# uc-vision/splat-trainer

Hardware: AMD Instinct MI355X
Metric: fwd+bwd Gaussians/s (higher is better)
Workload: dtype f32

## Files before the change

### splat-trainer_amd/csrc/ssim.hip

```cpp
#include "gsr_device.h"
#include "gsr_host.h"

namespace {

constexpr int TS = 32;
constexpr int HALO = 5;
constexpr int IN = TS + 2 * HALO;

struct Gauss11 {
  float w[11];
};

struct Strides {
  int64_t sB, sC, sH, sW;
};

__device__ __forceinline__ float clamp_keep_nan(float v, float lo, float hi) {
  return v < lo ? lo : (v > hi ? hi : v);
}

__device__ __forceinline__ float block_sum_256(float v, float* s_red) {
  v = gsr_wave_sum(v);
  const int wave = threadIdx.x >> 6;
  if ((threadIdx.x & 63) == 0) s_red[wave] = v;
  __syncthreads();
  return s_red[0] + s_red[1] + s_red[2] + s_red[3];
}

template <bool TRAIN>
__global__ __launch_bounds__(256) void ssim_fwd_kernel(const float* __restrict__ img1, const float* __restrict__ img2,
                                                       Strides st1, Strides st2, int C, int H, int W, int crop,
                                                       float C1, float C2, float inv_count, Gauss11 g,
                                                       float* __restrict__ block_sums, float* __restrict__ dm_dmu1,
                                                       float* __restrict__ dm_dm11, float* __restrict__ dm_dm12,
                                                       float lo = -INFINITY, float hi = INFINITY) {
  __shared__ float s_x[IN][IN + 1], s_y[IN][IN + 1];
  __shared__ float s_h[5][IN][TS + 1];
  __shared__ float s_red[4];
  const int plane = blockIdx.z, b = plane / C, c = plane % C;
  const int x0 = blockIdx.x * TS, y0 = blockIdx.y * TS;
  const float* p1 = img1 + b * st1.sB + c * st1.sC;
  const float* p2 = img2 + b * st2.sB + c * st2.sC;
  const int cy = min(y0 + TS / 2, H - 1), cx = min(x0 + TS / 2, W - 1);
  float c1 = clamp_keep_nan(p1[cy * st1.sH + cx * st1.sW], lo, hi), c2 = p2[cy * st2.sH + cx * st2.sW];
  c1 = fabsf(c1) <= 3.0e38f ? c1 : 0.f;
  c2 = fabsf(c2) <= 3.0e38f ? c2 : 0.f;
  for (int i = threadIdx.x; i < IN * IN; i += 256) {
    const int ly = i / IN, lx = i % IN;
    const int gy = y0 + ly - HALO, gx = x0 + lx - HALO;
    const bool in = gy >= 0 && gy < H && gx >= 0 && gx < W;
    s_x[ly][lx] = in ? clamp_keep_nan(p1[gy * st1.sH + gx * st1.sW], lo, hi) - c1 : 0.f;
    s_y[ly][lx] = in ? p2[gy * st2.sH + gx * st2.sW] - c2 : 0.f;
  }
  __syncthreads();
  for (int i = threadIdx.x; i < IN * (TS / 4); i += 256) {
    const int ly = i / (TS / 4), lx = (i % (TS / 4)) * 4;
    float x[14], y[14], xx[14], yy[14], xy[14];
#pragma unroll
    for (int k = 0; k < 14; ++k) {
      x[k] = s_x[ly][lx + k]; y[k] = s_y[ly][lx + k];
      xx[k] = x[k] * x[k]; yy[k] = y[k] * y[k]; xy[k] = x[k] * y[k];
    }
#pragma unroll
    for (int o = 0; o < 4; ++o) {
      float a = 0.f, bb = 0.f, aa = 0.f, bb2 = 0.f, ab = 0.f;
#pragma unroll
      for (int k = 0; k < 11; ++k) {
        const float w = g.w[k];
        a += w * x[o + k]; bb += w * y[o + k]; aa += w * xx[o + k]; bb2 += w * yy[o + k]; ab += w * xy[o + k];
      }
      s_h[0][ly][lx + o] = a; s_h[1][ly][lx + o] = bb; s_h[2][ly][lx + o] = aa; s_h[3][ly][lx + o] = bb2;
      s_h[4][ly][lx + o] = ab;
    }
  }
  __syncthreads();
  const int tx = threadIdx.x & 31, tg = threadIdx.x >> 5;
  const int gx = x0 + tx;
  float acc[4][5];
#pragma unroll
  for (int o = 0; o < 4; ++o)
#pragma unroll
    for (int q = 0; q < 5; ++q) acc[o][q] = 0.f;
#pragma unroll
  for (int q = 0; q < 5; ++q) {
    float col[14];
#pragma unroll
    for (int k = 0; k < 14; ++k) col[k] = s_h[q][tg * 4 + k][tx];
#pragma unroll
    for (int o = 0; o < 4; ++o)
#pragma unroll
      for (int k = 0; k < 11; ++k) acc[o][q] += g.w[k] * col[o + k];
  }
  float local = 0.f;
  float out_x = 0.f;
#pragma unroll
  for (int k = 0; k < 11; ++k) out_x += (gx + k - HALO < 0 || gx + k - HALO >= W) ? g.w[k] : 0.f;
#pragma unroll
  for (int o = 0; o < 4; ++o) {
    const int gy = y0 + tg * 4 + o;
    float out_y = 0.f;
#pragma unroll
    for (int k = 0; k < 11; ++k) out_y += (gy + k - HALO < 0 || gy + k - HALO >= H) ? g.w[k] : 0.f;
    const float mass = (1.f - out_x) * (1.f - out_y), rest = out_x + (1.f - out_x) * out_y;
    const float n1 = acc[o][0], n2 = acc[o][1];
    const float mu1 = n1 + c1 * mass, mu2 = n2 + c2 * mass;
    const float s1 = (acc[o][2] - n1 * n1) + c1 * rest * (2.f * n1 + c1 * mass);
    const float s2 = (acc[o][3] - n2 * n2) + c2 * rest * (2.f * n2 + c2 * mass);
    const float s12 = (acc[o][4] - n1 * n2) + rest * (c2 * n1 + c1 * n2 + c1 * c2 * mass);
    const bool inside = gx < W && gy < H;
    const bool counted = inside && gx >= crop && gx < W - crop && gy >= crop && gy < H - crop;
    const float A1 = 2.f * mu1 * mu2 + C1, A2 = 2.f * s12 + C2;
    const float B1 = mu1 * mu1 + mu2 * mu2 + C1, B2 = s1 + s2 + C2;
    const float iB = 1.f / (B1 * B2);
    if (counted) local += A1 * A2 * iB;
    if (TRAIN && inside) {
      const float sc = counted ? inv_count : 0.f;
      const float d_mu1 = 2.f * mu2 * (A2 - A1) * iB - 2.f * mu1 * A1 * A2 * (B2 - B1) * iB * iB;
      const float d_m11 = -A1 * A2 * iB / B2;
      const float d_m12 = 2.f * A1 * iB;
      const int64_t oidx = ((int64_t)plane * H + gy) * W + gx;
      dm_dmu1[oidx] = sc * d_mu1; dm_dm11[oidx] = sc * d_m11; dm_dm12[oidx] = sc * d_m12;
    }
  }
  const float total = block_sum_256(local, s_red);
  if (threadIdx.x == 0)
    block_sums[(blockIdx.z * gridDim.y + blockIdx.y) * gridDim.x + blockIdx.x] = total;
}

__global__ __launch_bounds__(256) void ssim_finish_kernel(const float* __restrict__ block_sums, int n, float inv_count,
                                                          float* __restrict__ out) {
  __shared__ float s_red[4];
  float acc = 0.f;
  for (int i = threadIdx.x; i < n; i += 256) acc += block_sums[i];
  const float total = block_sum_256(acc, s_red);
  if (threadIdx.x == 0) out[0] = total * inv_count;
}

__global__ __launch_bounds__(256) void ssim_bwd_kernel(const float* __restrict__ img1, const float* __restrict__ img2,
                                                       Strides st1, Strides st2, Strides sto, int C, int H, int W,
                                                       Gauss11 g, const float* __restrict__ dm_dmu1,
                                                       const float* __restrict__ dm_dm11,
                                                       const float* __restrict__ dm_dm12,
                                                       const float* __restrict__ gscale_dev, float* __restrict__ dimg1,
                                                       float lo = -INFINITY, float hi = INFINITY) {
  __shared__ float s_in[3][IN][IN + 1];
  __shared__ float s_h[3][IN][TS + 1];
  const int plane = blockIdx.z, b = plane / C, c = plane % C;
  const int x0 = blockIdx.x * TS, y0 = blockIdx.y * TS;
  const int64_t pbase = (int64_t)plane * H * W;
  for (int i = threadIdx.x; i < IN * IN; i += 256) {
    const int ly = i / IN, lx = i % IN;
    const int gy = y0 + ly - HALO, gx = x0 + lx - HALO;
    const bool in = gy >= 0 && gy < H && gx >= 0 && gx < W;
    const int64_t o = pbase + (int64_t)gy * W + gx;
    s_in[0][ly][lx] = in ? dm_dmu1[o] : 0.f;
    s_in[1][ly][lx] = in ? dm_dm11[o] : 0.f;
    s_in[2][ly][lx] = in ? dm_dm12[o] : 0.f;
  }
  __syncthreads();
  for (int i = threadIdx.x; i < IN * (TS / 4); i += 256) {
    const int ly = i / (TS / 4), lx = (i % (TS / 4)) * 4;
#pragma unroll
    for (int q = 0; q < 3; ++q) {
      float v[14];
#pragma unroll
      for (int k = 0; k < 14; ++k) v[k] = s_in[q][ly][lx + k];
#pragma unroll
      for (int o = 0; o < 4; ++o) {
        float a = 0.f;
#pragma unroll
        for (int k = 0; k < 11; ++k) a += g.w[k] * v[o + k];
        s_h[q][ly][lx + o] = a;
      }
    }
  }
  __syncthreads();
  const int tx = threadIdx.x & 31, tg = threadIdx.x >> 5;
  const int gx = x0 + tx;
  float acc[4][3];
#pragma unroll
  for (int q = 0; q < 3; ++q) {
    float col[14];
#pragma unroll
    for (int k = 0; k < 14; ++k) col[k] = s_h[q][tg * 4 + k][tx];
#pragma unroll
    for (int o = 0; o < 4; ++o) {
      float a = 0.f;
#pragma unroll
      for (int k = 0; k < 11; ++k) a += g.w[k] * col[o + k];
      acc[o][q] = a;
    }
  }
  if (gx >= W) return;
  const float gs = gscale_dev ? gscale_dev[0] : 1.f;
#pragma unroll
  for (int o = 0; o < 4; ++o) {
    const int gy = y0 + tg * 4 + o;
    if (gy >= H) continue;
    const float x = clamp_keep_nan(img1[b * st1.sB + c * st1.sC + gy * st1.sH + gx * st1.sW], lo, hi);
    const float y = img2[b * st2.sB + c * st2.sC + gy * st2.sH + gx * st2.sW];
    dimg1[b * sto.sB + c * sto.sC + gy * sto.sH + gx * sto.sW] = gs * (acc[o][0] + 2.f * x * acc[o][1] + y * acc[o][2]);
  }
}

Gauss11 make_gauss() {
  Gauss11 g;
  double sum = 0.0, w[11];
  for (int i = 0; i < 11; ++i) { const double d = i - 5; w[i] = exp(-(d * d) / (2.0 * 1.5 * 1.5)); sum += w[i]; }
  for (int i = 0; i < 11; ++i) g.w[i] = (float)(w[i] / sum);
  return g;
}

constexpr int PL_THREADS = 256;
constexpr int PL_ITEMS = 8;

template <int KIND>
__global__ __launch_bounds__(PL_THREADS) void pixel_loss_fwd_kernel(const float* __restrict__ x,
                                                                    const float* __restrict__ t, int64_t n, float lo,
                                                                    float hi, float* __restrict__ block_sums) {
  __shared__ float s_w[PL_THREADS / 64];
  float acc = 0.f;
  for (int64_t i = ((int64_t)blockIdx.x * PL_THREADS + threadIdx.x) * 4; i < n; i += (int64_t)gridDim.x * PL_THREADS * 4) {
    float xv[4], tv[4];
    if (i + 3 < n) {
      const float4 a = *reinterpret_cast<const float4*>(x + i), b = *reinterpret_cast<const float4*>(t + i);
      xv[0] = a.x; xv[1] = a.y; xv[2] = a.z; xv[3] = a.w; tv[0] = b.x; tv[1] = b.y; tv[2] = b.z; tv[3] = b.w;
    } else {
#pragma unroll
      for (int k = 0; k < 4; ++k) { xv[k] = i + k < n ? x[i + k] : 0.f; tv[k] = i + k < n ? t[i + k] : clamp_keep_nan(0.f, lo, hi); }
    }
#pragma unroll
    for (int k = 0; k < 4; ++k) {
      const float d = clamp_keep_nan(xv[k], lo, hi) - tv[k];
      acc += KIND == 0 ? d * d : fabsf(d);
    }
  }
  acc = gsr_wave_sum(acc);
  if (gsr_lane() == 0) s_w[threadIdx.x >> 6] = acc;
  __syncthreads();
  if (threadIdx.x == 0) block_sums[blockIdx.x] = (s_w[0] + s_w[1]) + (s_w[2] + s_w[3]);
}

__global__ __launch_bounds__(256) void pixel_loss_finish_kernel(const float* __restrict__ block_sums, int blocks,
                                                                float inv_n, float* __restrict__ out) {
  __shared__ float s_w[4];
  float acc = 0.f;
  for (int b = threadIdx.x; b < blocks; b += 256) acc += block_sums[b];
  acc = gsr_wave_sum(acc);
  if (gsr_lane() == 0) s_w[threadIdx.x >> 6] = acc;
  __syncthreads();
  if (threadIdx.x == 0) out[0] = ((s_w[0] + s_w[1]) + (s_w[2] + s_w[3])) * inv_n;
}

template <int KIND>
__global__ __launch_bounds__(PL_THREADS) void pixel_loss_bwd_kernel(const float* __restrict__ x,
                                                                    const float* __restrict__ t, int64_t n, float lo,
                                                                    float hi, float inv_n,
                                                                    const float* __restrict__ grad_scale,
                                                                    float* __restrict__ dx) {
  const float gs = grad_scale[0] * inv_n;
  for (int64_t i = (int64_t)blockIdx.x * PL_THREADS + threadIdx.x; i < n; i += (int64_t)gridDim.x * PL_THREADS) {
    const float xv = x[i];
    const float d = clamp_keep_nan(xv, lo, hi) - t[i];
    const bool pass = xv >= lo && xv <= hi;
    const float g = KIND == 0 ? 2.f * d : (d > 0.f ? 1.f : (d < 0.f ? -1.f : 0.f));
    dx[i] = pass ? gs * g : 0.f;
  }
}

constexpr int ML_MAX_LEVELS = 4;

struct MsLevels {
  int n;
  int H[ML_MAX_LEVELS], W[ML_MAX_LEVELS];
  float* pred[ML_MAX_LEVELS];
  float* targ[ML_MAX_LEVELS];
  float* dlev[ML_MAX_LEVELS];
};

__global__ __launch_bounds__(256) void msloss_pyramid_kernel(const float* __restrict__ image,
                                                             const float* __restrict__ target, int C, MsLevels lv,
                                                             float lo, float hi, float* __restrict__ block_l1,
                                                             float* __restrict__ block_mse) {
  __shared__ float s_a[4], s_b[4];
  const int H = lv.H[0], W = lv.W[0];
  const int bw = (W + 7) / 8, bh = (H + 7) / 8;
  const int64_t id = (int64_t)blockIdx.x * 256 + threadIdx.x;
  float l1 = 0.f, mse = 0.f;
  if (id < (int64_t)bw * bh * C) {
    const int c = (int)(id % C);
    const int bx = (int)((id / C) % bw), by = (int)(id / ((int64_t)C * bw));
    float x1[4][4], t1[4][4];
#pragma unroll
    for (int j = 0; j < 4; ++j)
#pragma unroll
      for (int i = 0; i < 4; ++i) {
        float sx = 0.f, st = 0.f;
#pragma unroll
        for (int dy = 0; dy < 2; ++dy)
#pragma unroll
          for (int dx = 0; dx < 2; ++dx) {
            const int y = by * 8 + 2 * j + dy, x = bx * 8 + 2 * i + dx;
            if (y < H && x < W) {
              const int64_t o = ((int64_t)y * W + x) * C + c;
              const float xv = clamp_keep_nan(image[o], lo, hi), tv = target[o];
              const float d = xv - tv;
              l1 += fabsf(d);
              mse += d * d;
              sx += xv; st += tv;
            }
          }
        x1[j][i] = 0.25f * sx; t1[j][i] = 0.25f * st;
        const int y1 = by * 4 + j, xq = bx * 4 + i;
        if (lv.n > 1 && y1 < lv.H[1] && xq < lv.W[1]) {
          const int64_t o = ((int64_t)y1 * lv.W[1] + xq) * C + c;
          lv.pred[1][o] = x1[j][i]; lv.targ[1][o] = t1[j][i];
        }
      }
    if (lv.n > 2) {
      float x2[2][2], t2[2][2];
#pragma unroll
      for (int j = 0; j < 2; ++j)
#pragma unroll
        for (int i = 0; i < 2; ++i) {
          x2[j][i] = 0.25f * ((x1[2 * j][2 * i] + x1[2 * j][2 * i + 1]) + (x1[2 * j + 1][2 * i] + x1[2 * j + 1][2 * i + 1]));
          t2[j][i] = 0.25f * ((t1[2 * j][2 * i] + t1[2 * j][2 * i + 1]) + (t1[2 * j + 1][2 * i] + t1[2 * j + 1][2 * i + 1]));
          const int y2 = by * 2 + j, xq = bx * 2 + i;
          if (y2 < lv.H[2] && xq < lv.W[2]) {
            const int64_t o = ((int64_t)y2 * lv.W[2] + xq) * C + c;
            lv.pred[2][o] = x2[j][i]; lv.targ[2][o] = t2[j][i];
          }
        }
      if (lv.n > 3 && by < lv.H[3] && bx < lv.W[3]) {
        const int64_t o = ((int64_t)by * lv.W[3] + bx) * C + c;
        lv.pred[3][o] = 0.25f * ((x2[0][0] + x2[0][1]) + (x2[1][0] + x2[1][1]));
        lv.targ[3][o] = 0.25f * ((t2[0][0] + t2[0][1]) + (t2[1][0] + t2[1][1]));
      }
    }
  }
  l1 = gsr_wave_sum(l1);
  mse = gsr_wave_sum(mse);
  if (gsr_lane() == 0) { s_a[threadIdx.x >> 6] = l1; s_b[threadIdx.x >> 6] = mse; }
  __syncthreads();
  if (threadIdx.x == 0) {
    block_l1[blockIdx.x] = (s_a[0] + s_a[1]) + (s_a[2] + s_a[3]);
    block_mse[blockIdx.x] = (s_b[0] + s_b[1]) + (s_b[2] + s_b[3]);
  }
}

struct MsSums {
  const float* ssim[ML_MAX_LEVELS];
  int ssim_n[ML_MAX_LEVELS];
  float ssim_inv[ML_MAX_LEVELS];
  const float* l1;
  const float* mse;
  int pix_n;
  float pix_inv;
};

__global__ __launch_bounds__(256) void msloss_finish_kernel(MsSums sm, int levels, float w_l1, float w_mse, float w_ssim,
                                                            float* __restrict__ metrics_out) {
  __shared__ float s_red[4];
  float vals[2 + ML_MAX_LEVELS];
  float a = 0.f;
  for (int i = threadIdx.x; i < sm.pix_n; i += 256) a += sm.l1[i];
  vals[0] = block_sum_256(a, s_red) * sm.pix_inv;
  __syncthreads();
  a = 0.f;
  for (int i = threadIdx.x; i < sm.pix_n; i += 256) a += sm.mse[i];
  vals[1] = block_sum_256(a, s_red) * sm.pix_inv;
  __syncthreads();
  float ssim_loss = 0.f;
  for (int l = 0; l < levels; ++l) {
    a = 0.f;
    for (int i = threadIdx.x; i < sm.ssim_n[l]; i += 256) a += sm.ssim[l][i];
    vals[2 + l] = block_sum_256(a, s_red) * sm.ssim_inv[l];
    __syncthreads();
    ssim_loss += 1.f - vals[2 + l];
  }
  if (threadIdx.x == 0) {
    metrics_out[0] = vals[0] * w_l1 + vals[1] * w_mse + (ssim_loss / (float)levels) * w_ssim;
    for (int k = 0; k < 2 + levels; ++k) metrics_out[1 + k] = vals[k];
  }
}

__global__ __launch_bounds__(256) void msloss_combine_kernel(const float* __restrict__ image,
                                                             const float* __restrict__ target, int C, MsLevels lv,
                                                             float lo, float hi, float w_l1, float w_mse, float w_ssim,
                                                             const float* __restrict__ up, float* __restrict__ d_image) {
  const int H = lv.H[0], W = lv.W[0];
  const int64_t n = (int64_t)H * W * C;
  const float inv_n = 1.f / (float)n, gs = up[0], cs = -w_ssim / (float)lv.n;
  for (int64_t i = (int64_t)blockIdx.x * 256 + threadIdx.x; i < n; i += (int64_t)gridDim.x * 256) {
    const float xv = image[i];
    if (!(xv >= lo && xv <= hi)) { d_image[i] = 0.f; continue; }
    const int c = (int)(i % C);
    const int64_t p = i / C;
    const int x = (int)(p % W), y = (int)(p / W);
    const float d = xv - target[i];
    float g = w_l1 * inv_n * (d > 0.f ? 1.f : (d < 0.f ? -1.f : 0.f)) + w_mse * inv_n * 2.f * d;
    float s = d_image[i], sc = 0.25f;
#pragma unroll
    for (int l = 1; l < ML_MAX_LEVELS; ++l) {
      if (l < lv.n) {
        const int yl = y >> l, xl = x >> l;
        if (yl < lv.H[l] && xl < lv.W[l]) s += sc * lv.dlev[l][((int64_t)yl * lv.W[l] + xl) * C + c];
        sc *= 0.25f;
      }
    }
    d_image[i] = gs * (g + cs * s);
  }
}

struct MsPlan {
  MsLevels lv;
  size_t maps[ML_MAX_LEVELS];
  size_t sums[ML_MAX_LEVELS];
  int sums_n[ML_MAX_LEVELS];
  size_t pix_l1, pix_mse;
  int pix_blocks;
  size_t total;
};

MsPlan ms_plan(int H, int W, int C, int levels, uint8_t* base) {
  MsPlan p;
  size_t at = 0;
  auto take = [&](size_t bytes) { const size_t o = at; at = (at + bytes + 255) / 256 * 256; return o; };
  p.lv.n = levels;
  int h = H, w = W;
  for (int l = 0; l < ML_MAX_LEVELS; ++l) {
    p.lv.H[l] = p.lv.W[l] = 0;
    p.lv.pred[l] = p.lv.targ[l] = p.lv.dlev[l] = nullptr;
    p.maps[l] = p.sums[l] = 0; p.sums_n[l] = 0;
    if (l >= levels) continue;
    if (l > 0) { h /= 2; w /= 2; }
    p.lv.H[l] = h; p.lv.W[l] = w;
    const size_t plane = (size_t)h * w * C * sizeof(float);
    if (l > 0) {
      p.lv.pred[l] = reinterpret_cast<float*>(base + take(plane));
      p.lv.targ[l] = reinterpret_cast<float*>(base + take(plane));
      p.lv.dlev[l] = reinterpret_cast<float*>(base + take(plane));
    }
    p.maps[l] = take(3 * plane);
    p.sums_n[l] = ((w + TS - 1) / TS) * ((h + TS - 1) / TS) * C;
    p.sums[l] = take((size_t)p.sums_n[l] * sizeof(float));
  }
  const int64_t work = (int64_t)((W + 7) / 8) * ((H + 7) / 8) * C;
  p.pix_blocks = (int)((work + 255) / 256);
  p.pix_l1 = take((size_t)p.pix_blocks * sizeof(float));
  p.pix_mse = take((size_t)p.pix_blocks * sizeof(float));
  p.total = at;
  return p;
}

inline bool ms_args_ok(int H, int W, int C, int levels) {
  if (H <= 0 || W <= 0 || C < 1 || C > 4 || levels < 1 || levels > ML_MAX_LEVELS) return false;
  return (H >> (levels - 1)) > 10 && (W >> (levels - 1)) > 10;
}

}

extern "C" {

size_t gsr_ssim_workspace_bytes(int32_t B, int32_t C, int32_t H, int32_t W) {
  if (B <= 0 || C <= 0 || H <= 0 || W <= 0) return 256;
  const size_t blocks = (size_t)((W + TS - 1) / TS) * ((H + TS - 1) / TS) * B * C;
  return blocks * sizeof(float) + 256;
}

int gsr_ssim_forward(const float* img1, const float* img2, const int64_t* strides1_host, const int64_t* strides2_host,
                     int32_t B, int32_t C, int32_t H, int32_t W, int32_t crop, float* mean_out, float* dm_dmu1,
                     float* dm_dm11, float* dm_dm12, void* workspace, size_t workspace_bytes, void* stream_) {
  hipStream_t stream = gsr_stream(stream_);
  if (B <= 0 || C <= 0 || H <= 0 || W <= 0 || crop < 0 || !img1 || !img2 || !mean_out || !strides1_host || !strides2_host)
    return GSR_ERR_INVALID_ARGUMENT;
  if (W - 2 * crop <= 0 || H - 2 * crop <= 0) return GSR_ERR_INVALID_ARGUMENT;
  if (!workspace || workspace_bytes < gsr_ssim_workspace_bytes(B, C, H, W)) return GSR_ERR_WORKSPACE_TOO_SMALL;
  const bool train = dm_dmu1 && dm_dm11 && dm_dm12;
  const Strides s1 = {strides1_host[0], strides1_host[1], strides1_host[2], strides1_host[3]};
  const Strides s2 = {strides2_host[0], strides2_host[1], strides2_host[2], strides2_host[3]};
  const dim3 grid((W + TS - 1) / TS, (H + TS - 1) / TS, B * C);
  const int nblocks = grid.x * grid.y * grid.z;
  const float inv_count = 1.f / ((float)B * C * (H - 2 * crop) * (float)(W - 2 * crop));
  float* block_sums = reinterpret_cast<float*>(workspace);
  const Gauss11 g = make_gauss();
  gsr_pick_bool(train, [&](auto tr) {
    ssim_fwd_kernel<decltype(tr)::value><<<grid, 256, 0, stream>>>(
        img1, img2, s1, s2, C, H, W, crop, 0.01f * 0.01f, 0.03f * 0.03f, inv_count, g, block_sums,
        train ? dm_dmu1 : nullptr, train ? dm_dm11 : nullptr, train ? dm_dm12 : nullptr);
  });
  GSR_CHECK_LAUNCH();
  ssim_finish_kernel<<<1, 256, 0, stream>>>(block_sums, nblocks, inv_count, mean_out);
  GSR_CHECK_LAUNCH();
  return GSR_OK;
}

int gsr_ssim_backward(const float* img1, const float* img2, const int64_t* strides1_host, const int64_t* strides2_host,
                      const int64_t* strides_out_host, int32_t B, int32_t C, int32_t H, int32_t W, const float* dm_dmu1,
                      const float* dm_dm11, const float* dm_dm12, const float* grad_scale_dev, float* d_img1,
                      void* stream_) {
  hipStream_t stream = gsr_stream(stream_);
  if (B <= 0 || C <= 0 || H <= 0 || W <= 0 || !img1 || !img2 || !dm_dmu1 || !dm_dm11 || !dm_dm12 || !grad_scale_dev ||
      !d_img1 || !strides1_host || !strides2_host || !strides_out_host)
    return GSR_ERR_INVALID_ARGUMENT;
  const Strides s1 = {strides1_host[0], strides1_host[1], strides1_host[2], strides1_host[3]};
  const Strides s2 = {strides2_host[0], strides2_host[1], strides2_host[2], strides2_host[3]};
  const Strides so = {strides_out_host[0], strides_out_host[1], strides_out_host[2], strides_out_host[3]};
  const dim3 grid((W + TS - 1) / TS, (H + TS - 1) / TS, B * C);
  ssim_bwd_kernel<<<grid, 256, 0, stream>>>(img1, img2, s1, s2, so, C, H, W, make_gauss(), dm_dmu1, dm_dm11, dm_dm12,
                                           grad_scale_dev, d_img1);
  GSR_CHECK_LAUNCH();
  return GSR_OK;
}

size_t gsr_msloss_workspace_bytes(int32_t H, int32_t W, int32_t C, int32_t levels) {
  if (!ms_args_ok(H, W, C, levels)) return 256;
  return ms_plan(H, W, C, levels, nullptr).total + 256;
}

int gsr_msloss_forward(const float* image, const float* target, int32_t H, int32_t W, int32_t C, int32_t levels,
                       float w_l1, float w_mse, float w_ssim, float lo, float hi, float* metrics_out, void* workspace,
                       size_t workspace_bytes, void* stream_) {
  hipStream_t stream = gsr_stream(stream_);
  if (!ms_args_ok(H, W, C, levels) || !image || !target || !metrics_out || !(lo <= hi)) return GSR_ERR_INVALID_ARGUMENT;
  if (!workspace || workspace_bytes < gsr_msloss_workspace_bytes(H, W, C, levels)) return GSR_ERR_WORKSPACE_TOO_SMALL;
  uint8_t* base = reinterpret_cast<uint8_t*>(workspace);
  const MsPlan p = ms_plan(H, W, C, levels, base);
  msloss_pyramid_kernel<<<p.pix_blocks, 256, 0, stream>>>(image, target, C, p.lv, lo, hi,
                                                         reinterpret_cast<float*>(base + p.pix_l1),
                                                         reinterpret_cast<float*>(base + p.pix_mse));
  GSR_CHECK_LAUNCH();
  const Gauss11 g = make_gauss();
  MsSums sm;
  for (int l = 0; l < ML_MAX_LEVELS; ++l) { sm.ssim[l] = nullptr; sm.ssim_n[l] = 0; sm.ssim_inv[l] = 0.f; }
  for (int l = 0; l < levels; ++l) {
    const int h = p.lv.H[l], w = p.lv.W[l];
    const Strides st = {0, 1, (int64_t)w * C, C};
    const float* x = l ? p.lv.pred[l] : image;
    const float* t = l ? p.lv.targ[l] : target;
    const dim3 grid((w + TS - 1) / TS, (h + TS - 1) / TS, C);
    const float inv_count = 1.f / ((float)C * (h - 10) * (float)(w - 10));
    float* maps = reinterpret_cast<float*>(base + p.maps[l]);
    const size_t plane = (size_t)h * w * C;
    ssim_fwd_kernel<true><<<grid, 256, 0, stream>>>(x, t, st, st, C, h, w, 5, 0.01f * 0.01f, 0.03f * 0.03f, inv_count, g,
                                                   reinterpret_cast<float*>(base + p.sums[l]), maps, maps + plane,
                                                   maps + 2 * plane, l ? -INFINITY : lo, l ? INFINITY : hi);
    GSR_CHECK_LAUNCH();
    sm.ssim[l] = reinterpret_cast<const float*>(base + p.sums[l]);
    sm.ssim_n[l] = p.sums_n[l];
    sm.ssim_inv[l] = inv_count;
  }
  sm.l1 = reinterpret_cast<const float*>(base + p.pix_l1);
  sm.mse = reinterpret_cast<const float*>(base + p.pix_mse);
  sm.pix_n = p.pix_blocks;
  sm.pix_inv = 1.f / ((float)H * (float)W * (float)C);
  msloss_finish_kernel<<<1, 256, 0, stream>>>(sm, levels, w_l1, w_mse, w_ssim, metrics_out);
  GSR_CHECK_LAUNCH();
  return GSR_OK;
}

int gsr_msloss_backward(const float* image, const float* target, int32_t H, int32_t W, int32_t C, int32_t levels,
                        float w_l1, float w_mse, float w_ssim, float lo, float hi, const float* grad_scale_dev,
                        void* workspace, size_t workspace_bytes, float* d_image, void* stream_) {
  hipStream_t stream = gsr_stream(stream_);
  if (!ms_args_ok(H, W, C, levels) || !image || !target || !grad_scale_dev || !d_image) return GSR_ERR_INVALID_ARGUMENT;
  if (!workspace || workspace_bytes < gsr_msloss_workspace_bytes(H, W, C, levels)) return GSR_ERR_WORKSPACE_TOO_SMALL;
  uint8_t* base = reinterpret_cast<uint8_t*>(workspace);
  const MsPlan p = ms_plan(H, W, C, levels, base);
  const Gauss11 g = make_gauss();
  for (int l = 0; l < levels; ++l) {
    const int h = p.lv.H[l], w = p.lv.W[l];
    const Strides st = {0, 1, (int64_t)w * C, C};
    const float* x = l ? p.lv.pred[l] : image;
    const float* t = l ? p.lv.targ[l] : target;
    const float* maps = reinterpret_cast<const float*>(base + p.maps[l]);
    const size_t plane = (size_t)h * w * C;
    const dim3 grid((w + TS - 1) / TS, (h + TS - 1) / TS, C);
    ssim_bwd_kernel<<<grid, 256, 0, stream>>>(x, t, st, st, st, C, h, w, g, maps, maps + plane, maps + 2 * plane, nullptr,
                                             l ? p.lv.dlev[l] : d_image, l ? -INFINITY : lo, l ? INFINITY : hi);
    GSR_CHECK_LAUNCH();
  }
  const int64_t n = (int64_t)H * W * C;
  const int64_t want = (n + 255) / 256;
  msloss_combine_kernel<<<(int)(want < 16384 ? want : 16384), 256, 0, stream>>>(image, target, C, p.lv, lo, hi, w_l1, w_mse,
                                                                              w_ssim, grad_scale_dev, d_image);
  GSR_CHECK_LAUNCH();
  return GSR_OK;
}

size_t gsr_pixel_loss_workspace_bytes(int64_t n) {
  const int64_t blocks = (n + (int64_t)PL_THREADS * 4 - 1) / ((int64_t)PL_THREADS * 4);
  return (size_t)(blocks < 1024 ? (blocks < 1 ? 1 : blocks) : 1024) * sizeof(float) + 256;
}

int gsr_pixel_loss_forward(const float* image, const float* target, int64_t n, int32_t kind, float lo, float hi,
                           float* loss_out, void* workspace, size_t workspace_bytes, void* stream_) {
  hipStream_t stream = gsr_stream(stream_);
  if (n <= 0 || !image || !target || !loss_out || (kind != 0 && kind != 1) || !(lo <= hi)) return GSR_ERR_INVALID_ARGUMENT;
  if (!workspace || workspace_bytes < gsr_pixel_loss_workspace_bytes(n)) return GSR_ERR_WORKSPACE_TOO_SMALL;
  if ((reinterpret_cast<uintptr_t>(image) | reinterpret_cast<uintptr_t>(target)) & 15) return GSR_ERR_INVALID_ARGUMENT;
  const int64_t want = (n + (int64_t)PL_THREADS * 4 - 1) / ((int64_t)PL_THREADS * 4);
  const int blocks = (int)(want < 1024 ? want : 1024);
  float* sums = reinterpret_cast<float*>(workspace);
  gsr_pick<0, 1>(kind, [&](auto k) {
    pixel_loss_fwd_kernel<decltype(k)::value><<<blocks, PL_THREADS, 0, stream>>>(image, target, n, lo, hi, sums);
  });
  pixel_loss_finish_kernel<<<1, 256, 0, stream>>>(sums, blocks, 1.f / (float)n, loss_out);
  GSR_CHECK_LAUNCH();
  return GSR_OK;
}

int gsr_pixel_loss_backward(const float* image, const float* target, int64_t n, int32_t kind, float lo, float hi,
                            const float* grad_scale_dev, float* d_image, void* stream_) {
  hipStream_t stream = gsr_stream(stream_);
  if (n <= 0 || !image || !target || !grad_scale_dev || !d_image || (kind != 0 && kind != 1)) return GSR_ERR_INVALID_ARGUMENT;
  const int64_t want = (n + PL_THREADS - 1) / PL_THREADS;
  const int blocks = (int)(want < 8192 ? want : 8192);
  gsr_pick<0, 1>(kind, [&](auto k) {
    pixel_loss_bwd_kernel<decltype(k)::value><<<blocks, PL_THREADS, 0, stream>>>(image, target, n, lo, hi, 1.f / (float)n,
                                                                                grad_scale_dev, d_image);
  });
  GSR_CHECK_LAUNCH();
  return GSR_OK;
}

}
```

Baseline: 585.1 million.

## Batch SSIM levels into single launches with packed float2 filtering and reduced LDS

New measurement: 583.8 million. No clear change (-0.2%).

```diff
diff --git a/splat-trainer_amd/csrc/ssim.hip b/splat-trainer_amd/csrc/ssim.hip
--- a/splat-trainer_amd/csrc/ssim.hip
+++ b/splat-trainer_amd/csrc/ssim.hip
@@ -6,6 +6,7 @@
 constexpr int TS = 32;
 constexpr int HALO = 5;
 constexpr int IN = TS + 2 * HALO;
+constexpr int ML_MAX_LEVELS = 4;
 
 struct Gauss11 {
   float w[11];
@@ -27,86 +28,233 @@
   return s_red[0] + s_red[1] + s_red[2] + s_red[3];
 }
 
+struct SsimLevel {
+  const float* img1;
+  const float* img2;
+  Strides st1, st2, sto;
+  float* dm_dmu1;
+  float* dm_dm11;
+  float* dm_dm12;
+  float* block_sums;
+  float* dimg1;
+  int C, H, W, crop, tiles_x, tiles_y, units, per_die;
+  float inv_count, lo, hi;
+};
+
+struct SsimBatch {
+  int n;
+  int first[ML_MAX_LEVELS + 1];
+  SsimLevel lv[ML_MAX_LEVELS];
+};
+
+struct SsimTile {
+  int l, plane, x0, y0, sum_at;
+  bool valid;
+};
+
+constexpr int DIES = 8;
+__device__ __forceinline__ SsimTile ssim_tile(const SsimBatch& bt) {
+  SsimTile t;
+  const int b = blockIdx.x;
+  t.l = 0;
+#pragma unroll
+  for (int l = 1; l < ML_MAX_LEVELS; ++l)
+    if (l < bt.n && b >= bt.first[l]) t.l = l;
+  const SsimLevel& L = bt.lv[t.l];
+  const int tiles = L.tiles_x * L.tiles_y;
+  const int j = b - bt.first[t.l], k = j / DIES;
+  const int slot = k / L.C, c = k - slot * L.C;
+  const int unit = (j % DIES) * L.per_die + slot;
+  const int batch = unit / tiles, tile = unit - batch * tiles;
+  t.valid = unit < L.units;
+  t.plane = batch * L.C + c;
+  t.sum_at = t.plane * tiles + tile;
+  t.y0 = (tile / L.tiles_x) * TS;
+  t.x0 = (tile % L.tiles_x) * TS;
+  return t;
+}
+
+typedef float v2f __attribute__((ext_vector_type(2)));
+
+__device__ __forceinline__ void taps4_pair(const Gauss11& g, const v2f (&v)[14], v2f (&out)[4]) {
+#pragma unroll
+  for (int o = 0; o < 4; ++o) {
+    v2f a = {0.f, 0.f};
+#pragma unroll
+    for (int k = 0; k < 11; ++k) a = __builtin_elementwise_fma(v2f{g.w[k], g.w[k]}, v[o + k], a);
+    out[o] = a;
+  }
+}
+
+__device__ __forceinline__ void taps4_single(const Gauss11& g, const float (&v)[14], float (&out)[4]) {
+#pragma unroll
+  for (int o = 0; o < 4; o += 2) {
+    v2f a = {fmaf(g.w[0], v[o], 0.f), 0.f};
+#pragma unroll
+    for (int s = 1; s < 11; ++s) {
+      float both = v[o + s];
+      asm("" : "+v"(both));
+      a = __builtin_elementwise_fma(v2f{g.w[s], g.w[s - 1]}, v2f{both, both}, a);
+    }
+    out[o] = a.x;
+    out[o + 1] = fmaf(g.w[10], v[o + 11], a.y);
+  }
+}
+
+constexpr int XS = IN + 1;
+template <int STAGED, int PAIRS, int ODD>
+struct TilePlan {
+  static constexpr int staged = IN * XS * STAGED;
+  static constexpr int raw_row = (2 * PAIRS + ODD) * (TS + 1);
+  static constexpr int ROW = raw_row + ((6 - raw_row % 32) + 32) % 32;
+  static constexpr int low = TS * ROW;
+  static constexpr int high_at = staged > low ? staged : low;
+  static constexpr int total = high_at + (IN - TS) * ROW;
+  __device__ static __forceinline__ int row(int r) { return r < TS ? r * ROW : high_at + (r - TS) * ROW; }
+};
+using FwdPlan = TilePlan<2, 2, 1>;
+using BwdPlan = TilePlan<3, 1, 1>;
+static_assert(FwdPlan::ROW % 2 == 0 && BwdPlan::ROW % 2 == 0 && FwdPlan::high_at % 2 == 0 && BwdPlan::high_at % 2 == 0,
+              "float2 accesses need even offsets");
+
+__device__ __forceinline__ void hpass_item(int i, int& ly, int& lx) {
+  if (i < 256) { ly = i & 31; lx = (i >> 5) * 4; }
+  else { ly = TS + (i - 256) % (IN - TS); lx = ((i - 256) / (IN - TS)) * 4; }
+}
+
+constexpr int STAGE_ROWS = 6, STAGE_ROUNDS = IN / STAGE_ROWS;
+static_assert(STAGE_ROWS * STAGE_ROUNDS == IN && STAGE_ROWS * IN <= 256, "the staging rounds cover the tile exactly");
+struct StageItem {
+  int lx, row, gx;
+  bool active, col_in;
+};
+__device__ __forceinline__ StageItem stage_item(int x0, int W) {
+  StageItem s;
+  s.row = threadIdx.x / IN;
+  s.lx = threadIdx.x - s.row * IN;
+  s.gx = x0 + s.lx - HALO;
+  s.active = threadIdx.x < STAGE_ROWS * IN;
+  s.col_in = s.active && s.gx >= 0 && s.gx < W;
+  return s;
+}
+
 template <bool TRAIN>
-__global__ __launch_bounds__(256) void ssim_fwd_kernel(const float* __restrict__ img1, const float* __restrict__ img2,
-                                                       Strides st1, Strides st2, int C, int H, int W, int crop,
-                                                       float C1, float C2, float inv_count, Gauss11 g,
-                                                       float* __restrict__ block_sums, float* __restrict__ dm_dmu1,
-                                                       float* __restrict__ dm_dm11, float* __restrict__ dm_dm12,
-                                                       float lo = -INFINITY, float hi = INFINITY) {
-  __shared__ float s_x[IN][IN + 1], s_y[IN][IN + 1];
-  __shared__ float s_h[5][IN][TS + 1];
+__global__ __launch_bounds__(256, 5) void ssim_fwd_kernel(SsimBatch bt, float C1, float C2, Gauss11 g) {
+  using P = FwdPlan;
+  __shared__ __attribute__((aligned(16))) float s_f[P::total];
   __shared__ float s_red[4];
-  const int plane = blockIdx.z, b = plane / C, c = plane % C;
-  const int x0 = blockIdx.x * TS, y0 = blockIdx.y * TS;
-  const float* p1 = img1 + b * st1.sB + c * st1.sC;
-  const float* p2 = img2 + b * st2.sB + c * st2.sC;
+  v2f* s_xy = reinterpret_cast<v2f*>(s_f);
+  const SsimTile tl = ssim_tile(bt);
+  if (!tl.valid) return;
+  const SsimLevel& L = bt.lv[tl.l];
+  const Strides st1 = L.st1, st2 = L.st2;
+  const int C = L.C, H = L.H, W = L.W, crop = L.crop;
+  const float lo = L.lo, hi = L.hi, inv_count = L.inv_count;
+  const int plane = tl.plane, b = plane / C, c = plane % C;
+  const int x0 = tl.x0, y0 = tl.y0;
+  const float* p1 = L.img1 + b * st1.sB + c * st1.sC;
+  const float* p2 = L.img2 + b * st2.sB + c * st2.sC;
   const int cy = min(y0 + TS / 2, H - 1), cx = min(x0 + TS / 2, W - 1);
-  float c1 = clamp_keep_nan(p1[cy * st1.sH + cx * st1.sW], lo, hi), c2 = p2[cy * st2.sH + cx * st2.sW];
+  const int64_t centre1 = cy * st1.sH + cx * st1.sW, centre2 = cy * st2.sH + cx * st2.sW;
+  const StageItem si = stage_item(x0, W);
+  const int64_t at1 = (y0 + si.row - HALO) * st1.sH + si.gx * st1.sW, at2 = (y0 + si.row - HALO) * st2.sH + si.gx * st2.sW;
+  float raw1[STAGE_ROUNDS], raw2[STAGE_ROUNDS];
+#pragma unroll
+  for (int r = 0; r < STAGE_ROUNDS; ++r) {
+    const int gy = y0 + si.row + STAGE_ROWS * r - HALO;
+    const bool in = si.col_in && gy >= 0 && gy < H;
+    raw1[r] = p1[in ? at1 + r * STAGE_ROWS * st1.sH : centre1];
+    raw2[r] = p2[in ? at2 + r * STAGE_ROWS * st2.sH : centre2];
+  }
+  float c1 = clamp_keep_nan(p1[centre1], lo, hi), c2 = p2[centre2];
   c1 = fabsf(c1) <= 3.0e38f ? c1 : 0.f;
   c2 = fabsf(c2) <= 3.0e38f ? c2 : 0.f;
-  for (int i = threadIdx.x; i < IN * IN; i += 256) {
-    const int ly = i / IN, lx = i % IN;
-    const int gy = y0 + ly - HALO, gx = x0 + lx - HALO;
-    const bool in = gy >= 0 && gy < H && gx >= 0 && gx < W;
-    s_x[ly][lx] = in ? clamp_keep_nan(p1[gy * st1.sH + gx * st1.sW], lo, hi) - c1 : 0.f;
-    s_y[ly][lx] = in ? p2[gy * st2.sH + gx * st2.sW] - c2 : 0.f;
-  }
-  __syncthreads();
-  for (int i = threadIdx.x; i < IN * (TS / 4); i += 256) {
-    const int ly = i / (TS / 4), lx = (i % (TS / 4)) * 4;
-    float x[14], y[14], xx[14], yy[14], xy[14];
-#pragma unroll
-    for (int k = 0; k < 14; ++k) {
-      x[k] = s_x[ly][lx + k]; y[k] = s_y[ly][lx + k];
-      xx[k] = x[k] * x[k]; yy[k] = y[k] * y[k]; xy[k] = x[k] * y[k];
-    }
+#pragma unroll
+  for (int r = 0; r < STAGE_ROUNDS; ++r) {
+    const int gy = y0 + si.row + STAGE_ROWS * r - HALO;
+    const bool in = si.col_in && gy >= 0 && gy < H;
+    v2f v = {0.f, 0.f};
+    if (in) {
+      v.x = clamp_keep_nan(raw1[r], lo, hi) - c1;
+      v.y = raw2[r] - c2;
+    }
+    if (si.active) s_xy[(si.row + STAGE_ROWS * r) * XS + si.lx] = v;
+  }
+  __syncthreads();
+  auto hpass = [&](int ly, int lx, const v2f (&v)[14]) {
+    v2f sq[14], m[4], q[4];
+    float xy[14], cr[4];
+#pragma unroll
+    for (int k = 0; k < 14; ++k) { sq[k] = v[k] * v[k]; xy[k] = v[k].x * v[k].y; }
+    taps4_pair(g, v, m);
+    taps4_pair(g, sq, q);
+    taps4_single(g, xy, cr);
+    float* row = s_f + P::row(ly);
 #pragma unroll
     for (int o = 0; o < 4; ++o) {
-      float a = 0.f, bb = 0.f, aa = 0.f, bb2 = 0.f, ab = 0.f;
-#pragma unroll
-      for (int k = 0; k < 11; ++k) {
-        const float w = g.w[k];
-        a += w * x[o + k]; bb += w * y[o + k]; aa += w * xx[o + k]; bb2 += w * yy[o + k]; ab += w * xy[o + k];
-      }
-      s_h[0][ly][lx + o] = a; s_h[1][ly][lx + o] = bb; s_h[2][ly][lx + o] = aa; s_h[3][ly][lx + o] = bb2;
-      s_h[4][ly][lx + o] = ab;
-    }
-  }
-  __syncthreads();
+      reinterpret_cast<v2f*>(row)[lx + o] = m[o];
+      reinterpret_cast<v2f*>(row)[(TS + 1) + lx + o] = q[o];
+      row[4 * (TS + 1) + lx + o] = cr[o];
+    }
+  };
+  v2f in[14];
+  int ly, lx;
+  if (threadIdx.x < IN * (TS / 4) - 256) {
+    hpass_item(256 + threadIdx.x, ly, lx);
+#pragma unroll
+    for (int k = 0; k < 14; ++k) in[k] = s_xy[ly * XS + lx + k];
+    hpass(ly, lx, in);
+  }
+  hpass_item(threadIdx.x, ly, lx);
+#pragma unroll
+  for (int k = 0; k < 14; ++k) in[k] = s_xy[ly * XS + lx + k];
+  __syncthreads();
+  hpass(ly, lx, in);
   const int tx = threadIdx.x & 31, tg = threadIdx.x >> 5;
   const int gx = x0 + tx;
-  float acc[4][5];
-#pragma unroll
-  for (int o = 0; o < 4; ++o)
-#pragma unroll
-    for (int q = 0; q < 5; ++q) acc[o][q] = 0.f;
-#pragma unroll
-  for (int q = 0; q < 5; ++q) {
-    float col[14];
-#pragma unroll
-    for (int k = 0; k < 14; ++k) col[k] = s_h[q][tg * 4 + k][tx];
-#pragma unroll
-    for (int o = 0; o < 4; ++o)
-#pragma unroll
-      for (int k = 0; k < 11; ++k) acc[o][q] += g.w[k] * col[o + k];
+  __syncthreads();
+  v2f accm[4], accq[4];
+  float accc[4];
+  {
+    v2f col[14];
+#pragma unroll
+    for (int k = 0; k < 14; ++k) col[k] = reinterpret_cast<const v2f*>(s_f + P::row(tg * 4 + k))[tx];
+    taps4_pair(g, col, accm);
+#pragma unroll
+    for (int k = 0; k < 14; ++k) col[k] = reinterpret_cast<const v2f*>(s_f + P::row(tg * 4 + k))[(TS + 1) + tx];
+    taps4_pair(g, col, accq);
+    float one[14];
+#pragma unroll
+    for (int k = 0; k < 14; ++k) one[k] = s_f[P::row(tg * 4 + k) + 4 * (TS + 1) + tx];
+    taps4_single(g, one, accc);
+  }
+#pragma unroll
+  for (int o = 0; o < 4; ++o) asm volatile("" : "+v"(accm[o]), "+v"(accq[o]), "+v"(accc[o]));
+  const bool x_edge = x0 < HALO || x0 + TS + HALO > W, y_edge = y0 < HALO || y0 + TS + HALO > H;
+  float out_x = 0.f, out_ys[4] = {0.f, 0.f, 0.f, 0.f};
+  if (x_edge) {
+#pragma unroll
+    for (int k = 0; k < 11; ++k) out_x += (gx + k - HALO < 0 || gx + k - HALO >= W) ? g.w[k] : 0.f;
+  }
+  if (y_edge) {
+#pragma unroll
+    for (int o = 0; o < 4; ++o) {
+      const int gy = y0 + tg * 4 + o;
+#pragma unroll
+      for (int k = 0; k < 11; ++k) out_ys[o] += (gy + k - HALO < 0 || gy + k - HALO >= H) ? g.w[k] : 0.f;
+    }
   }
   float local = 0.f;
-  float out_x = 0.f;
-#pragma unroll
-  for (int k = 0; k < 11; ++k) out_x += (gx + k - HALO < 0 || gx + k - HALO >= W) ? g.w[k] : 0.f;
 #pragma unroll
   for (int o = 0; o < 4; ++o) {
     const int gy = y0 + tg * 4 + o;
-    float out_y = 0.f;
-#pragma unroll
-    for (int k = 0; k < 11; ++k) out_y += (gy + k - HALO < 0 || gy + k - HALO >= H) ? g.w[k] : 0.f;
+    const float out_y = out_ys[o];
     const float mass = (1.f - out_x) * (1.f - out_y), rest = out_x + (1.f - out_x) * out_y;
-    const float n1 = acc[o][0], n2 = acc[o][1];
+    const float n1 = accm[o].x, n2 = accm[o].y;
     const float mu1 = n1 + c1 * mass, mu2 = n2 + c2 * mass;
-    const float s1 = (acc[o][2] - n1 * n1) + c1 * rest * (2.f * n1 + c1 * mass);
-    const float s2 = (acc[o][3] - n2 * n2) + c2 * rest * (2.f * n2 + c2 * mass);
-    const float s12 = (acc[o][4] - n1 * n2) + rest * (c2 * n1 + c1 * n2 + c1 * c2 * mass);
+    const float s1 = (accq[o].x - n1 * n1) + c1 * rest * (2.f * n1 + c1 * mass);
+    const float s2 = (accq[o].y - n2 * n2) + c2 * rest * (2.f * n2 + c2 * mass);
+    const float s12 = (accc[o] - n1 * n2) + rest * (c2 * n1 + c1 * n2 + c1 * c2 * mass);
     const bool inside = gx < W && gy < H;
     const bool counted = inside && gx >= crop && gx < W - crop && gy >= crop && gy < H - crop;
     const float A1 = 2.f * mu1 * mu2 + C1, A2 = 2.f * s12 + C2;
@@ -119,12 +267,11 @@
       const float d_m11 = -A1 * A2 * iB / B2;
       const float d_m12 = 2.f * A1 * iB;
       const int64_t oidx = ((int64_t)plane * H + gy) * W + gx;
-      dm_dmu1[oidx] = sc * d_mu1; dm_dm11[oidx] = sc * d_m11; dm_dm12[oidx] = sc * d_m12;
+      L.dm_dmu1[oidx] = sc * d_mu1; L.dm_dm11[oidx] = sc * d_m11; L.dm_dm12[oidx] = sc * d_m12;
     }
   }
   const float total = block_sum_256(local, s_red);
-  if (threadIdx.x == 0)
-    block_sums[(blockIdx.z * gridDim.y + blockIdx.y) * gridDim.x + blockIdx.x] = total;
+  if (threadIdx.x == 0) L.block_sums[tl.sum_at] = total;
 }
 
 __global__ __launch_bounds__(256) void ssim_finish_kernel(const float* __restrict__ block_sums, int n, float inv_count,
@@ -136,70 +283,93 @@
   if (threadIdx.x == 0) out[0] = total * inv_count;
 }
 
-__global__ __launch_bounds__(256) void ssim_bwd_kernel(const float* __restrict__ img1, const float* __restrict__ img2,
-                                                       Strides st1, Strides st2, Strides sto, int C, int H, int W,
-                                                       Gauss11 g, const float* __restrict__ dm_dmu1,
-                                                       const float* __restrict__ dm_dm11,
-                                                       const float* __restrict__ dm_dm12,
-                                                       const float* __restrict__ gscale_dev, float* __restrict__ dimg1,
-                                                       float lo = -INFINITY, float hi = INFINITY) {
-  __shared__ float s_in[3][IN][IN + 1];
-  __shared__ float s_h[3][IN][TS + 1];
-  const int plane = blockIdx.z, b = plane / C, c = plane % C;
-  const int x0 = blockIdx.x * TS, y0 = blockIdx.y * TS;
+__global__ __launch_bounds__(256, 6) void ssim_bwd_kernel(SsimBatch bt, Gauss11 g, const float* __restrict__ gscale_dev) {
+  using P = BwdPlan;
+  __shared__ __attribute__((aligned(16))) float s_f[P::total];
+  v2f* s_ab = reinterpret_cast<v2f*>(s_f);
+  float* s_c = s_f + 2 * IN * XS;
+  const SsimTile tl = ssim_tile(bt);
+  if (!tl.valid) return;
+  const SsimLevel& L = bt.lv[tl.l];
+  const int C = L.C, H = L.H, W = L.W;
+  const int plane = tl.plane, b = plane / C, c = plane % C;
+  const int x0 = tl.x0, y0 = tl.y0;
   const int64_t pbase = (int64_t)plane * H * W;
-  for (int i = threadIdx.x; i < IN * IN; i += 256) {
-    const int ly = i / IN, lx = i % IN;
-    const int gy = y0 + ly - HALO, gx = x0 + lx - HALO;
-    const bool in = gy >= 0 && gy < H && gx >= 0 && gx < W;
-    const int64_t o = pbase + (int64_t)gy * W + gx;
-    s_in[0][ly][lx] = in ? dm_dmu1[o] : 0.f;
-    s_in[1][ly][lx] = in ? dm_dm11[o] : 0.f;
-    s_in[2][ly][lx] = in ? dm_dm12[o] : 0.f;
-  }
-  __syncthreads();
-  for (int i = threadIdx.x; i < IN * (TS / 4); i += 256) {
-    const int ly = i / (TS / 4), lx = (i % (TS / 4)) * 4;
-#pragma unroll
-    for (int q = 0; q < 3; ++q) {
-      float v[14];
-#pragma unroll
-      for (int k = 0; k < 14; ++k) v[k] = s_in[q][ly][lx + k];
-#pragma unroll
-      for (int o = 0; o < 4; ++o) {
-        float a = 0.f;
-#pragma unroll
-        for (int k = 0; k < 11; ++k) a += g.w[k] * v[o + k];
-        s_h[q][ly][lx + o] = a;
-      }
-    }
-  }
+  const float* __restrict__ dm_dmu1 = L.dm_dmu1;
+  const float* __restrict__ dm_dm11 = L.dm_dm11;
+  const float* __restrict__ dm_dm12 = L.dm_dm12;
+  const StageItem si = stage_item(x0, W);
+  const int64_t at = pbase + (int64_t)(y0 + si.row - HALO) * W + si.gx, safe = pbase + (int64_t)y0 * W + x0;
+  float ra[STAGE_ROUNDS], rb[STAGE_ROUNDS], rc[STAGE_ROUNDS];
+#pragma unroll
+  for (int r = 0; r < STAGE_ROUNDS; ++r) {
+    const int gy = y0 + si.row + STAGE_ROWS * r - HALO;
+    const int64_t o = (si.col_in && gy >= 0 && gy < H) ? at + (int64_t)r * STAGE_ROWS * W : safe;
+    ra[r] = dm_dmu1[o]; rb[r] = dm_dm11[o]; rc[r] = dm_dm12[o];
+  }
+#pragma unroll
+  for (int r = 0; r < STAGE_ROUNDS; ++r) {
+    const int gy = y0 + si.row + STAGE_ROWS * r - HALO;
+    const bool in = si.col_in && gy >= 0 && gy < H;
+    if (si.active) {
+      s_ab[(si.row + STAGE_ROWS * r) * XS + si.lx] = in ? v2f{ra[r], rb[r]} : v2f{0.f, 0.f};
+      s_c[(si.row + STAGE_ROWS * r) * XS + si.lx] = in ? rc[r] : 0.f;
+    }
+  }
+  __syncthreads();
+  auto hpass = [&](int ly, int lx, const v2f (&v)[14], const float (&w)[14]) {
+    v2f m[4];
+    float s[4];
+    taps4_pair(g, v, m);
+    taps4_single(g, w, s);
+    float* row = s_f + P::row(ly);
+#pragma unroll
+    for (int o = 0; o < 4; ++o) {
+      reinterpret_cast<v2f*>(row)[lx + o] = m[o];
+      row[2 * (TS + 1) + lx + o] = s[o];
+    }
+  };
+  v2f in2[14];
+  float in1[14];
+  int ly, lx;
+  if (threadIdx.x < IN * (TS / 4) - 256) {
+    hpass_item(256 + threadIdx.x, ly, lx);
+#pragma unroll
+    for (int k = 0; k < 14; ++k) { in2[k] = s_ab[ly * XS + lx + k]; in1[k] = s_c[ly * XS + lx + k]; }
+    hpass(ly, lx, in2, in1);
+  }
+  hpass_item(threadIdx.x, ly, lx);
+#pragma unroll
+  for (int k = 0; k < 14; ++k) { in2[k] = s_ab[ly * XS + lx + k]; in1[k] = s_c[ly * XS + lx + k]; }
+  __syncthreads();
+  hpass(ly, lx, in2, in1);
   __syncthreads();
   const int tx = threadIdx.x & 31, tg = threadIdx.x >> 5;
   const int gx = x0 + tx;
-  float acc[4][3];
-#pragma unroll
-  for (int q = 0; q < 3; ++q) {
-    float col[14];
-#pragma unroll
-    for (int k = 0; k < 14; ++k) col[k] = s_h[q][tg * 4 + k][tx];
-#pragma unroll
-    for (int o = 0; o < 4; ++o) {
-      float a = 0.f;
-#pragma unroll
-      for (int k = 0; k < 11; ++k) a += g.w[k] * col[o + k];
-      acc[o][q] = a;
-    }
+  v2f acc01[4];
+  float acc2[4];
+  {
+    v2f col[14];
+    float one[14];
+#pragma unroll
+    for (int k = 0; k < 14; ++k) {
+      col[k] = reinterpret_cast<const v2f*>(s_f + P::row(tg * 4 + k))[tx];
+      one[k] = s_f[P::row(tg * 4 + k) + 2 * (TS + 1) + tx];
+    }
+    taps4_pair(g, col, acc01);
+    taps4_single(g, one, acc2);
   }
   if (gx >= W) return;
   const float gs = gscale_dev ? gscale_dev[0] : 1.f;
+  const Strides st1 = L.st1, st2 = L.st2, sto = L.sto;
+  const float lo = L.lo, hi = L.hi;
 #pragma unroll
   for (int o = 0; o < 4; ++o) {
     const int gy = y0 + tg * 4 + o;
     if (gy >= H) continue;
-    const float x = clamp_keep_nan(img1[b * st1.sB + c * st1.sC + gy * st1.sH + gx * st1.sW], lo, hi);
-    const float y = img2[b * st2.sB + c * st2.sC + gy * st2.sH + gx * st2.sW];
-    dimg1[b * sto.sB + c * sto.sC + gy * sto.sH + gx * sto.sW] = gs * (acc[o][0] + 2.f * x * acc[o][1] + y * acc[o][2]);
+    const float x = clamp_keep_nan(L.img1[b * st1.sB + c * st1.sC + gy * st1.sH + gx * st1.sW], lo, hi);
+    const float y = L.img2[b * st2.sB + c * st2.sC + gy * st2.sH + gx * st2.sW];
+    L.dimg1[b * sto.sB + c * sto.sC + gy * sto.sH + gx * sto.sW] = gs * (acc01[o].x + 2.f * x * acc01[o].y + y * acc2[o]);
   }
 }
 
@@ -209,6 +379,17 @@
   for (int i = 0; i < 11; ++i) { const double d = i - 5; w[i] = exp(-(d * d) / (2.0 * 1.5 * 1.5)); sum += w[i]; }
   for (int i = 0; i < 11; ++i) g.w[i] = (float)(w[i] / sum);
   return g;
+}
+
+void ssim_batch_add(SsimBatch& bt, SsimLevel lv, int planes) {
+  lv.tiles_x = (lv.W + TS - 1) / TS;
+  lv.tiles_y = (lv.H + TS - 1) / TS;
+  lv.units = lv.tiles_x * lv.tiles_y * (planes / lv.C);
+  lv.per_die = (lv.units + DIES - 1) / DIES;
+  if (bt.n == 0) bt.first[0] = 0;
+  bt.lv[bt.n] = lv;
+  bt.first[bt.n + 1] = bt.first[bt.n] + DIES * lv.per_die * lv.C;
+  ++bt.n;
 }
 
 constexpr int PL_THREADS = 256;
@@ -267,8 +448,6 @@
     dx[i] = pass ? gs * g : 0.f;
   }
 }
-
-constexpr int ML_MAX_LEVELS = 4;
 
 struct MsLevels {
   int n;
@@ -458,6 +637,29 @@
   return (H >> (levels - 1)) > 10 && (W >> (levels - 1)) > 10;
 }
 
+SsimBatch ms_batch(const MsPlan& p, uint8_t* base, const float* image, const float* target, int C, float lo, float hi,
+                   float* d_image) {
+  SsimBatch bt = {};
+  for (int l = 0; l < p.lv.n; ++l) {
+    const int h = p.lv.H[l], w = p.lv.W[l];
+    const Strides st = {0, 1, (int64_t)w * C, C};
+    float* maps = reinterpret_cast<float*>(base + p.maps[l]);
+    const size_t plane = (size_t)h * w * C;
+    SsimLevel lv = {};
+    lv.img1 = l ? p.lv.pred[l] : image;
+    lv.img2 = l ? p.lv.targ[l] : target;
+    lv.st1 = lv.st2 = lv.sto = st;
+    lv.dm_dmu1 = maps; lv.dm_dm11 = maps + plane; lv.dm_dm12 = maps + 2 * plane;
+    lv.block_sums = reinterpret_cast<float*>(base + p.sums[l]);
+    lv.dimg1 = l ? p.lv.dlev[l] : d_image;
+    lv.C = C; lv.H = h; lv.W = w; lv.crop = 5;
+    lv.inv_count = 1.f / ((float)C * (h - 10) * (float)(w - 10));
+    lv.lo = l ? -INFINITY : lo; lv.hi = l ? INFINITY : hi;
+    ssim_batch_add(bt, lv, C);
+  }
+  return bt;
+}
+
 }
 
 extern "C" {
@@ -479,18 +681,22 @@
   const bool train = dm_dmu1 && dm_dm11 && dm_dm12;
   const Strides s1 = {strides1_host[0], strides1_host[1], strides1_host[2], strides1_host[3]};
   const Strides s2 = {strides2_host[0], strides2_host[1], strides2_host[2], strides2_host[3]};
-  const dim3 grid((W + TS - 1) / TS, (H + TS - 1) / TS, B * C);
-  const int nblocks = grid.x * grid.y * grid.z;
   const float inv_count = 1.f / ((float)B * C * (H - 2 * crop) * (float)(W - 2 * crop));
   float* block_sums = reinterpret_cast<float*>(workspace);
-  const Gauss11 g = make_gauss();
+  SsimLevel lv = {};
+  lv.img1 = img1; lv.img2 = img2; lv.st1 = s1; lv.st2 = s2;
+  lv.dm_dmu1 = train ? dm_dmu1 : nullptr; lv.dm_dm11 = train ? dm_dm11 : nullptr; lv.dm_dm12 = train ? dm_dm12 : nullptr;
+  lv.block_sums = block_sums;
+  lv.C = C; lv.H = H; lv.W = W; lv.crop = crop;
+  lv.inv_count = inv_count; lv.lo = -INFINITY; lv.hi = INFINITY;
+  SsimBatch bt = {};
+  ssim_batch_add(bt, lv, B * C);
+  const int nblocks = bt.first[1], nsums = bt.lv[0].units * C;
   gsr_pick_bool(train, [&](auto tr) {
-    ssim_fwd_kernel<decltype(tr)::value><<<grid, 256, 0, stream>>>(
-        img1, img2, s1, s2, C, H, W, crop, 0.01f * 0.01f, 0.03f * 0.03f, inv_count, g, block_sums,
-        train ? dm_dmu1 : nullptr, train ? dm_dm11 : nullptr, train ? dm_dm12 : nullptr);
+    ssim_fwd_kernel<decltype(tr)::value><<<nblocks, 256, 0, stream>>>(bt, 0.01f * 0.01f, 0.03f * 0.03f, make_gauss());
   });
   GSR_CHECK_LAUNCH();
-  ssim_finish_kernel<<<1, 256, 0, stream>>>(block_sums, nblocks, inv_count, mean_out);
+  ssim_finish_kernel<<<1, 256, 0, stream>>>(block_sums, nsums, inv_count, mean_out);
   GSR_CHECK_LAUNCH();
   return GSR_OK;
 }
@@ -506,9 +712,15 @@
   const Strides s1 = {strides1_host[0], strides1_host[1], strides1_host[2], strides1_host[3]};
   const Strides s2 = {strides2_host[0], strides2_host[1], strides2_host[2], strides2_host[3]};
   const Strides so = {strides_out_host[0], strides_out_host[1], strides_out_host[2], strides_out_host[3]};
-  const dim3 grid((W + TS - 1) / TS, (H + TS - 1) / TS, B * C);
-  ssim_bwd_kernel<<<grid, 256, 0, stream>>>(img1, img2, s1, s2, so, C, H, W, make_gauss(), dm_dmu1, dm_dm11, dm_dm12,
-                                           grad_scale_dev, d_img1);
+  SsimLevel lv = {};
+  lv.img1 = img1; lv.img2 = img2; lv.st1 = s1; lv.st2 = s2; lv.sto = so;
+  lv.dm_dmu1 = const_cast<float*>(dm_dmu1); lv.dm_dm11 = const_cast<float*>(dm_dm11); lv.dm_dm12 = const_cast<float*>(dm_dm12);
+  lv.dimg1 = d_img1;
+  lv.C = C; lv.H = H; lv.W = W;
+  lv.lo = -INFINITY; lv.hi = INFINITY;
+  SsimBatch bt = {};
+  ssim_batch_add(bt, lv, B * C);
+  ssim_bwd_kernel<<<bt.first[1], 256, 0, stream>>>(bt, make_gauss(), grad_scale_dev);
   GSR_CHECK_LAUNCH();
   return GSR_OK;
 }
@@ -530,25 +742,15 @@
                                                          reinterpret_cast<float*>(base + p.pix_l1),
                                                          reinterpret_cast<float*>(base + p.pix_mse));
   GSR_CHECK_LAUNCH();
-  const Gauss11 g = make_gauss();
+  const SsimBatch bt = ms_batch(p, base, image, target, C, lo, hi, nullptr);
+  ssim_fwd_kernel<true><<<bt.first[levels], 256, 0, stream>>>(bt, 0.01f * 0.01f, 0.03f * 0.03f, make_gauss());
+  GSR_CHECK_LAUNCH();
   MsSums sm;
   for (int l = 0; l < ML_MAX_LEVELS; ++l) { sm.ssim[l] = nullptr; sm.ssim_n[l] = 0; sm.ssim_inv[l] = 0.f; }
   for (int l = 0; l < levels; ++l) {
-    const int h = p.lv.H[l], w = p.lv.W[l];
-    const Strides st = {0, 1, (int64_t)w * C, C};
-    const float* x = l ? p.lv.pred[l] : image;
-    const float* t = l ? p.lv.targ[l] : target;
-    const dim3 grid((w + TS - 1) / TS, (h + TS - 1) / TS, C);
-    const float inv_count = 1.f / ((float)C * (h - 10) * (float)(w - 10));
-    float* maps = reinterpret_cast<float*>(base + p.maps[l]);
-    const size_t plane = (size_t)h * w * C;
-    ssim_fwd_kernel<true><<<grid, 256, 0, stream>>>(x, t, st, st, C, h, w, 5, 0.01f * 0.01f, 0.03f * 0.03f, inv_count, g,
-                                                   reinterpret_cast<float*>(base + p.sums[l]), maps, maps + plane,
-                                                   maps + 2 * plane, l ? -INFINITY : lo, l ? INFINITY : hi);
-    GSR_CHECK_LAUNCH();
-    sm.ssim[l] = reinterpret_cast<const float*>(base + p.sums[l]);
+    sm.ssim[l] = bt.lv[l].block_sums;
     sm.ssim_n[l] = p.sums_n[l];
-    sm.ssim_inv[l] = inv_count;
+    sm.ssim_inv[l] = bt.lv[l].inv_count;
   }
   sm.l1 = reinterpret_cast<const float*>(base + p.pix_l1);
   sm.mse = reinterpret_cast<const float*>(base + p.pix_mse);
@@ -567,19 +769,9 @@
   if (!workspace || workspace_bytes < gsr_msloss_workspace_bytes(H, W, C, levels)) return GSR_ERR_WORKSPACE_TOO_SMALL;
   uint8_t* base = reinterpret_cast<uint8_t*>(workspace);
   const MsPlan p = ms_plan(H, W, C, levels, base);
-  const Gauss11 g = make_gauss();
-  for (int l = 0; l < levels; ++l) {
-    const int h = p.lv.H[l], w = p.lv.W[l];
-    const Strides st = {0, 1, (int64_t)w * C, C};
-    const float* x = l ? p.lv.pred[l] : image;
-    const float* t = l ? p.lv.targ[l] : target;
-    const float* maps = reinterpret_cast<const float*>(base + p.maps[l]);
-    const size_t plane = (size_t)h * w * C;
-    const dim3 grid((w + TS - 1) / TS, (h + TS - 1) / TS, C);
-    ssim_bwd_kernel<<<grid, 256, 0, stream>>>(x, t, st, st, st, C, h, w, g, maps, maps + plane, maps + 2 * plane, nullptr,
-                                             l ? p.lv.dlev[l] : d_image, l ? -INFINITY : lo, l ? INFINITY : hi);
-    GSR_CHECK_LAUNCH();
-  }
+  const SsimBatch bt = ms_batch(p, base, image, target, C, lo, hi, d_image);
+  ssim_bwd_kernel<<<bt.first[levels], 256, 0, stream>>>(bt, make_gauss(), nullptr);
+  GSR_CHECK_LAUNCH();
   const int64_t n = (int64_t)H * W * C;
   const int64_t want = (n + 255) / 256;
   msloss_combine_kernel<<<(int)(want < 16384 ? want : 16384), 256, 0, stream>>>(image, target, C, p.lv, lo, hi, w_l1, w_mse,
```
